# saugns/saugns

Measured on AMD Instinct MI355X. Metric: mono samples/sec/GPU @ N voices (depth-3 FM), higher is better.
Workload: dtype f32 (f64 table interpolation, u32 phase)

## Files before the change

saugns_amd/csrc/engine.cpp:

```cpp
#include <atomic>
#include "engine.h"
#include <algorithm>
#include <exception>
#include <chrono>
#include <stdio.h>
#include <stdlib.h>
#include <string.h>

namespace sauengine {

static const sauProgramIDArr g_no_ids = {0};

static uint64_t ms_to_samples(uint64_t ms, uint64_t srate, int *carry) {
	uint64_t t = ms * srate;
	if (carry) {
		t += *carry;
		*carry = (int)(t % 1000);
	}
	return t / 1000;
}

Engine::~Engine() { delete backend_; }

const char *tune_env(const char *name) {
// ... 210 lines not shown
							err.clear();
						}
					}
				}
				if (vn.shape >= 0) {
					const VoicePlan &sp = shapes_[vn.shape].plan;
					if (plan_check_) {
						VoicePlan chk;
						std::string e2;
						const bool ok = compile_voice_plan(st.ops, vn.carr_op, chk, e2);
						if (!ok || chk.op_ids != shape_ids_ || chk.steps.size() != sp.steps.size() ||
						    memcmp(chk.steps.data(), sp.steps.data(), sp.steps.size() * sizeof(Step)) != 0 ||
						    chk.wave_mask != wmask || chk.n_fast != sp.n_fast || chk.n_fast_full != sp.n_fast_full ||
						    chk.n_slots != sp.n_slots || chk.n_main != sp.n_main || chk.no_fast != sp.no_fast ||
						    chk.static_block != sp.static_block || chk.selfmod != sp.selfmod || chk.n_chain != sp.n_chain ||
						    chk.n_osc != sp.n_osc || chk.has_camods != sp.has_camods || chk.carr_local != sp.carr_local || chk.wide != sp.wide) {
							err = "plan cache: a cached plan differs from a fresh compile (SAU_AMD_PLAN_CHECK)";
							return false;
						}
					}
					vn.plan.steps.clear(); vn.plan.fast_ids.clear(); vn.plan.fast_ids_full.clear();
					vn.plan.op_ids = shape_ids_;
					vn.plan.carr_local = sp.carr_local; vn.plan.n_slots = sp.n_slots; vn.plan.n_main = sp.n_main;
					vn.plan.n_fast = sp.n_fast; vn.plan.n_fast_full = sp.n_fast_full; vn.plan.wave_mask = wmask;
					vn.plan.has_camods = sp.has_camods; vn.plan.no_fast = sp.no_fast; vn.plan.static_block = sp.static_block;
					vn.plan.selfmod = sp.selfmod; vn.plan.n_chain = sp.n_chain; vn.plan.n_osc = sp.n_osc; vn.plan.wide = sp.wide;
					vn.plan.ras_cub = false;
					for (uint32_t id : shape_ids_) if (st.ops[id].ras_cub_seen) vn.plan.ras_cub = true;
					vn.plan.n_steps = (uint32_t)sp.steps.size();
				} else if (!compile_voice_plan(st.ops, vn.carr_op, vn.plan, err)) {
					vn.plan.steps.clear();
					vn.plan.fast_ids.clear();
					vn.plan.fast_ids_full.clear();
					vn.plan.op_ids.clear();
					vn.plan.n_steps = 0;
					if (err != "voice carrier operator was never initialised")
						return false;
					err.clear();
				} else {
					vn.plan.n_steps = (uint32_t)vn.plan.steps.size();
				}
// ... 73 lines not shown
		const sauProgramIDArr *lst = m.mods[use];
		for (uint32_t i = 0; i < count(lst); ++i) {
			const uint32_t o = estimate_sum_levels(st, lst->ids[i], dep, varies, need, nest + 1);
			if (o > out) out = o;
		}
	}
	return out;
}

bool Engine::render_segment(uint32_t len, uint32_t offset, bool stereo, std::string &err) {
	std::vector<VoiceDesc> descs;
	std::vector<SegmentDesc::Stream> sdescs(streams_.size());
	uint32_t n_main = 1, n_fpool = 0, max_ops = 1, n_pan = 0, max_steps = 1, n_fast = 1, n_fast_full = 0;
	uint64_t wave_mask = 0;
	bool maybe_block = false, serial = false, may_scan = false, maybe_cub = false;
	uint32_t sum_levels = 0, n_chain_rows = 0, n_chain_slots = 0, n_inc_rows = 0, n_look_rows = 0, n_may_scan = 0;
	bool chain_rows_padded = false;
	for (size_t s = 0; s < streams_.size(); ++s) {
		Stream &st = streams_[s];
		SegmentDesc::Stream &sd = sdescs[s];
		sd.first_voice = (uint32_t)descs.size();
		sd.amp_scale = st.amp_scale;
		sd.write_len = 0;
		Lattice lat;
		lat.call_len = lat_call_;
		lat.e0 = st.since_event < seg_call_pos_ ? (uint32_t)st.since_event : seg_call_pos_;
		lat.span_left = lat_call_ - seg_call_pos_;
		uint32_t ev_left = 0xffffffffu;
		if (st.event < st.events.size()) {
			const uint32_t wt = st.events[st.event].wait - (st.event_pos - len);
// ... 31 lines not shown
			d.inc_base = 0; d.n_inc = 0;
			d.look_base = 0; d.n_look = 0;
			if (dyn) line_begin(carr.pan, out_len, false, 0.f, lat, 0);
			else line_skip(carr.pan, out_len, lat, 0);
			descs.push_back(d);
			if (out_len > sd.write_len) sd.write_len = out_len;
			n_main = std::max(n_main, vn.plan.n_main);
			if (!vn.plan.no_fast) n_fast = std::max(n_fast, vn.plan.n_fast);
			n_fpool = std::max(n_fpool, vn.plan.n_slots - vn.plan.n_main);
			max_ops = std::max(max_ops, (uint32_t)vn.plan.op_ids.size());
			max_steps = std::max(max_steps, vn.plan.n_steps);
			wave_mask |= vn.plan.wave_mask;
			bool voice_block = vn.plan.static_block;
			if (vn.plan.static_block || vn.plan.no_fast) maybe_block = true;
			if (vn.plan.selfmod) serial = true;
			if (vn.plan.ras_cub && loop_tails_) maybe_cub = true;
			for (uint32_t id : vn.plan.op_ids) {
				OpMirror &m = st.ops[id];
				if (m.goal_seen || (m.line_set & (1u << L_PMA))) { maybe_block = true; voice_block = true; }
				if (m.line_set & (1u << L_PMA)) serial = true;
				if (id != vn.carr_op && !m.time_inf) {
					if (m.time < run_len) maybe_block = true;
					m.time -= std::min(m.time, out_len);
				}
			}
			if (out_len < run_len) maybe_block = true;
			if (voice_block && !vn.plan.no_fast) {
				n_fast_full = std::max(n_fast_full, vn.plan.n_fast_full);
				may_scan = true;
				++n_may_scan;
// ... 64 lines not shown
	seg.streams = sdescs.data(); seg.n_streams = (uint32_t)sdescs.size();
	seg.n_slots = n_main + n_fpool; seg.n_main = n_main; seg.n_fast = n_fast; seg.n_fast_full = n_fast_full; seg.max_ops = max_ops; seg.n_pan_rows = n_pan;
	seg.max_steps = max_steps;
	seg.wave_mask = wave_mask;
	seg.maybe_block = maybe_block;
	seg.serial = serial;
	seg.maybe_cub = maybe_cub;
	seg.may_scan = may_scan;
	seg.sum_levels = sum_levels;
	seg.n_chain_rows = n_chain_rows;
	seg.n_chain_slots = n_chain_slots > n_chain_rows ? n_chain_slots : n_chain_rows;
	seg.n_inc_rows = n_inc_rows;
	seg.n_look_rows = n_look_rows;
	seg.n_may_scan = n_may_scan;
	seg.chain_rows_padded = chain_rows_padded;
	return backend_->render(seg, err);
}

bool Engine::reserve(size_t frames, bool stereo, std::string &err) {
	if (frames > UINT32_MAX) { err = "buffer too long"; return false; }
	if ((uint32_t)frames > reserved_frames_ || (stereo && !reserved_stereo_)) {
		const uint32_t want = std::max((uint32_t)frames, reserved_frames_);
		if (!backend_->reserve_frames(want, stereo || reserved_stereo_, err)) return false;
		reserved_frames_ = want;
		reserved_stereo_ = stereo || reserved_stereo_;
	}
	return true;
}

bool Engine::snapshot(Snapshot &s, int slot, std::string &err) {
// ... 297 lines not shown
```

saugns_amd/csrc/engine.h:

```cpp
#ifndef SAU_ENGINE_H
#define SAU_ENGINE_H

#include "../../include/sau_abi.h"
#include "sau_dev_types.h"
#include "sau_flac.h"
#include "sau_dither.h"
#include <stddef.h>
#include <stdint.h>
#include <stdlib.h>
#include <string>
#include <unordered_map>
#include <vector>

namespace sauengine {

using namespace saudev;

enum SampleFormat : uint8_t { SF_S16 = 0, SF_F32 = 1 };

struct Levels {
	uint64_t frames;
	float peak[2];
	double sum_sq[2];
	uint64_t over[2], full_scale[2], nonfinite[2];
// ... 131 lines not shown
	bool may_scan;
	uint32_t sum_levels = 2;
	uint32_t max_ops;
	uint32_t max_steps;
	uint32_t n_pan_rows;
	uint64_t wave_mask;
	bool maybe_block;
	bool serial;
	bool maybe_cub = false;
	uint32_t n_chain_rows = 0;
	uint32_t n_inc_rows = 0;
	uint32_t n_look_rows = 0;
	uint32_t n_may_scan = 0;
	uint32_t n_chain_slots = 0;
	bool chain_rows_padded = false;
};

inline size_t chain_rows_budget(size_t free_b, unsigned fails) {
	static const long long env_mb = [] {
		const char *v = getenv("SAU_AMD_CHAIN_ROWS_MB");
		return v ? atoll(v) : -1ll;
	}();
	const unsigned sh = fails > 40 ? 40 : fails;
	if (env_mb >= 0) return ((size_t)env_mb << 20) >> sh;
	const size_t dflt = (size_t)24 << 30;
	if (!free_b) return dflt >> sh;
	return (free_b / 8 < dflt ? free_b / 8 : dflt) >> sh;
}

struct BackendConfig {
// ... 163 lines not shown
	std::vector<uint32_t> op_ids;
	uint32_t carr_local = 0;
	uint32_t n_slots = 0;
	uint32_t n_main = 0;
	uint32_t n_fast = 0;
	std::vector<FastIds> fast_ids;
	uint32_t n_fast_full = 0;
	std::vector<FastIds> fast_ids_full;
	uint64_t wave_mask = 0;
	bool has_camods = false;
	bool no_fast = false;
	bool wide = false;
	bool static_block = false;
	bool selfmod = false;
	bool ras_cub = false;
	uint32_t n_chain = 0;
	uint32_t n_osc = 0;
};

bool compile_voice_plan(const std::vector<OpMirror> &ops, uint32_t carrier,
		VoicePlan &out, std::string &err);
bool voice_plan_shape(const std::vector<OpMirror> &ops, uint32_t carrier, std::vector<uint32_t> &tokens,
		std::vector<uint32_t> &op_ids, std::vector<uint32_t> &stamp, uint32_t mark, uint64_t &wave_mask);


constexpr uint32_t CHAIN_SEG = 131072;
const char *tune_env(const char *name);
uint32_t chain_seg_frames(size_t n_chains, size_t budget_bytes);

class Engine {
// ... 161 lines not shown
```

saugns_amd/csrc/hip_backend.hip:

```cpp
#include <hip/hip_runtime.h>
#include "hip_backend.h"
#include "launch_plan.h"
#include "sau_dev_ops.h"
#include "sau_md5.h"
#include <float.h>
#include <stdio.h>
#include <stdlib.h>
#include <string.h>
#include <deque>
#include <map>
#include <memory>
#include <mutex>
#include <string>
#include <type_traits>
#include <vector>

namespace sauhip {

using namespace saudev;
using sauengine::BackendConfig;
using sauengine::tune_env;
using sauengine::SegmentDesc;
using namespace sauplan;

// ... 139 lines not shown
}

static std::mutex &attr_mutex() { static std::mutex *m = new std::mutex; return *m; }
static bool raise_lds_attr(const void *fn, size_t lds, int dev, std::string &err) {
	static std::map<std::pair<const void *, int>, size_t> *slots = new std::map<std::pair<const void *, int>, size_t>;
	std::lock_guard<std::mutex> lk(attr_mutex());
	size_t &configured = (*slots)[std::make_pair(fn, dev & 15)];
	if (lds > configured) {
		hipError_t e = hipFuncSetAttribute(fn, hipFuncAttributeMaxDynamicSharedMemorySize, (int)lds);
		if (e != hipSuccess) { err = std::string("hipFuncSetAttribute: ") + hipGetErrorString(e); return false; }
		configured = lds;
	}
	return true;
}

enum : unsigned { FK_WIDE = 1, FK_TAIL = 2, FK_CUB = 4, FK_INNER = 8, FK_LANEMAJOR = 16, FK_TAB0 = 32 };
static const void *fast_kernel_fn(int build, uint32_t rows, unsigned form) {
	struct Entry { int build; uint32_t rows; unsigned form; const void *fn; };
#define FK(build, form, ...) {build, FK_ROWS(__VA_ARGS__), form, (const void *)fast_kernel<__VA_ARGS__>}
#define FK_ROWS(rows, ...) rows
	static const Entry table[] = {
		FK(0, 0, 2, 0), FK(0, 0, 4, 0), FK(0, 0, 5, 0), FK(0, 0, 6, 0), FK(0, 0, 8, 0),
		FK(1, 0, 2, 1), FK(1, 0, 4, 1),
		FK(2, 0, 2, 2), FK(2, 0, 4, 2), FK(2, 0, 5, 2), FK(2, 0, 6, 2), FK(2, 0, 8, 2),
		FK(3, 0, 4, 3), FK(3, 0, 5, 3), FK(3, 0, 6, 3),
		FK(0, FK_WIDE, 6, 0, false, true), FK(0, FK_WIDE, 8, 0, false, true), FK(0, FK_WIDE, 10, 0, false, true), FK(0, FK_WIDE, 12, 0, false, true),
		FK(2, FK_WIDE | FK_TAIL, 8, 2, false, true, true), FK(2, FK_WIDE, 8, 2, false, true), FK(2, FK_TAIL, 8, 2, false, false, true),
		FK(2, FK_CUB, (int)FAST_CUB_ROWS, 2, true),
		FK(0, FK_WIDE | FK_INNER | FK_LANEMAJOR, 12, 0, false, true, false, true, true), FK(0, FK_WIDE | FK_INNER, 12, 0, false, true, false, true),
#if FK_LM_TAB0
		FK(0, FK_WIDE | FK_INNER | FK_LANEMAJOR | FK_TAB0, 12, 0, false, true, false, true, true, true),
#endif
		FK(0, FK_CUB, (int)FAST_CUB_ROWS, 0, true)};
#undef FK
#undef FK_ROWS
	for (const Entry &e : table)
		if (e.build == build && e.rows == rows && e.form == form) return e.fn;
	return nullptr;
}
#if FK_LM_TAB0
static bool tab0_kernel_ok(const void *fn) {
	static const bool ok = [&] { hipFuncAttributes a; return fn && hipFuncGetAttributes(&a, fn) == hipSuccess && a.sharedSizeBytes == 0; }();
	return ok;
}
#endif
static const void *repair_kernel_fn(uint32_t rows, bool wide) {
// ... 746 lines not shown
			fp.inmix_div_s = k.div.s; fp.inmix_div_m = k.div.m;
			if (k.inmix) {
				fp.inmix_stream = sets_[j.set].mstreams.p;
				fp.inmix_pcm_offset = seg.pcm_offset;
				hipLaunchKernelGGL(premix_kernel, dim3((seg.n_voices + 63) / 64), dim3(64), 0, stream_, fp);
				j.inmix_live = true;
			}
		}
		if (k.inner != INNER_NONE) {
			const bool lm = k.inner == INNER_LANE_MAJOR;
#if FK_LM_TAB0
			const bool tab0 = lm && k.inner_tab0 && tab0_kernel_ok(fast_kernel_fn(0, 12, FK_WIDE | FK_INNER | FK_LANEMAJOR | FK_TAB0));
#else
			const bool tab0 = false;
#endif
			const void *ik = fast_kernel_fn(0, 12, FK_WIDE | FK_INNER | (lm ? FK_LANEMAJOR : 0u) | (tab0 ? FK_TAB0 : 0u));
			if (!ik) { err = "no inner instantiation of fast_kernel for this form"; return false; }
			const size_t lds = k.inner_lds();
			FastParams ep = fp;
			ep.mode = 0; ep.edge_only = 1; ep.dyn_static = 1; ep.dyn_chunks = 2; ep.dyn_small = 0; ep.inmix_flags = 0;
			if (!launch_build(j, err, 0, k.rows, k.grid_edge, &ep, false, true)) j.launched = false;
			fp.mode = 0;
			void *iargs[] = {(void *)&fp};
			if (!raise_lds_attr(ik, lds, dev_, err)) return false;
			if (fp.inmix_flags && !pcm_hazard(err)) return false;
			HIP_OK(hipLaunchKernel(ik, dim3(k.grid), dim3(1024), iargs, lds, stream_));
			if (inner_report_) fprintf(stderr, "[sau-amd] inner: %s, %u voices, %u tables%s\n", lm ? "lane-major" : "row-major", seg.n_voices, k.tabs.n, tab0 ? ", tab0" : "");
		} else {
			if (inner_report_) fprintf(stderr, "[sau-amd] inner: none (rows %u, wide %d, chunks %u), %u voices\n", k.rows, k.wide_cf ? 1 : 0, fp.dyn_chunks, seg.n_voices);
			if (fp.inmix_flags && (!rows_hazard(j, err) || !pcm_hazard(err))) return false;
			launch_fast(j, err, 0);
		}
		fp.dyn_chunks = 0; fp.inmix_flags = 0; fp.dyn_small = 0;
		return true;
	}

	bool launch_cub(Job &j, std::string &err) {
		if (!j.fp.cub_ok) return true;
		const FastPlan &k = j.fk;
		FastParams q = k.main_build == 2 ? j.cfp : j.fp;
		q.n_fast = k.n_fast_cf; q.rows = FAST_CUB_ROWS; q.mode = 0; q.only_multi = 0;
		q.dyn_chunks = k.tasks_cub.dyn_chunks; q.dyn_static = k.tasks_cub.dyn_static;
// ... 1617 lines not shown
```

saugns_amd/csrc/k_fast_group_lm.h:

```cpp
		const int j0 = l * T;
		const int t0 = (int)(cg * GF) - (int)H + j0;
		const uint32_t om = ((1u << T) - 1u) & ~((1u << min(max((int)H - j0, 0), T)) - 1u);
		auto prev32 = [&](const uint32_t *x, int k) -> uint32_t { return k > 0 ? x[k - 1] : lane_prev(x[T - 1]); };
		auto prev64 = [&](const double *x, int k) -> double { return k > 0 ? x[k - 1] : lane_prev(x[T - 1]); };
		const bool quads = ((cg * GF - H) & 3u) == 0;
		auto store_row = [&](float *row, const float *x, const bool nt) {
			uint32_t o = om;
			asm volatile("" : "+v"(o));
			if (quads) {
#pragma unroll
				for (int q = 0; q < T / 4; ++q) {
					const uint32_t oq = (o >> (4 * q)) & 15u;
					if (oq == 15u) {
						const fk_f32x4 v4 = {x[4 * q], x[4 * q + 1], x[4 * q + 2], x[4 * q + 3]};
						fk_f32x4 *p = (fk_f32x4 *)(row + t0 + 4 * q);
						if (nt) FK_VSTORE(p, v4); else *p = v4;
					} else if (oq != 0u) {
#pragma unroll
						for (int u = 0; u < 4; ++u)
							if ((oq >> u) & 1u) { if (nt) FK_VSTORE(&row[t0 + 4 * q + u], x[4 * q + u]); else row[t0 + 4 * q + u] = x[4 * q + u]; }
					}
				}
			} else {
#pragma unroll
				for (int k = 0; k < T; ++k)
					if ((o >> k) & 1u) { if (nt) FK_VSTORE(&row[t0 + k], x[k]); else row[t0 + k] = x[k]; }
			}
		};
		uint32_t held_rows = 0;
		bool held_far = false;
		float blk[T];
		for (uint32_t si = 0; si < n_fsteps; ++si) {
			const FastStep f = load_step_uniform(fsteps + si);
			const uint32_t kind = f.kind & 0xff;
			const uint32_t flags = (f.kind >> 8) & 0xff;
			int t0s = t0;
			asm volatile("" : "+v"(t0s));
			{
				const uint32_t o1 = f.out_off + 1u, p1 = f.pm_off + 1u, q1 = f.fpm_off + 1u, a1 = f.amp_off + 1u;
				uint32_t two = 0;
				if (kind == ST_OSC) two = o1 | a1 | (p1 + q1) | (flags & SF_WAVE_ENV);
				else if (kind == ST_LINE) two = o1;
				else if (kind == ST_VOICE) two = o1 | (p1 << 1);
				else if (kind == ST_LERP) two = 2u;
				if (two > 1u) { zero_acc = 1; continue; }
			}
			if (kind == ST_OSC) {
				const uint32_t type = f.type & 0xff;
				const bool layer = (flags & SF_LAYER) != 0;
				const bool to_voice = ((f.kind >> 16) & OX_VOICE) != 0;
				float s[T];
				if (type == OT_WAVE) {
					const bool has_pm = f.pm_off != ~0u, has_fpm = f.fpm_off != ~0u;
					const int p_min = (int)H - (int)(f.kind >> 24) + 1;
					const int nd = min(max(p_min - j0, 0), T);
					const uint32_t dm = ((1u << T) - 1u) & ~((1u << nd) - 1u);
					bool done = false;
					if (FK_COMMON && f.tab >= 0 && !has_fpm && !(f.ramp & 2)) {
						uint32_t ph[T];
						{
							uint32_t acc = f.phase0 + f.inc * (uint32_t)(t0 + 1);
#pragma unroll
							for (int k = 0; k < T; ++k) { ph[k] = acc; acc += f.inc; }
						}
						bool ok = true;
						if (has_pm) {
							float pm[T];
							bool big = false;
#pragma unroll
							for (int k = 0; k < T; ++k) {
								pm[k] = blk[k];
								big |= !(fabsf(pm[k]) < 0x1p20f);
							}
							ok = !__any(big);
#pragma unroll
							for (int k = 0; k < T; ++k) ph[k] += rint32w_p31_small(pm[k]);
						}
						if (ok) {
							const uint32_t ltab = tabs + (uint32_t)f.tab * FkTab<WIDE>::BYTES;
							static_assert(T % 2 == 0, "pairs of samples");
							auto hermite = [&](auto &&sink) {
// ... 177 lines not shown
								const int j = j0 + (int)__builtin_ctz(held);
								rep[1] = ((uint32_t)(j % 64 - p_min) << 24) | ((uint32_t)(j / 64) << 20) | (si << 12) | (cg & 0xfff);
							}
							const int nf = jm + p_min - j0;
							const bool far = nf <= 0 ? held != 0u : nf < T ? (held >> nf) != 0u : false;
							if (__any(far)) held_far = true;
							if (jm > 0) {
								unsigned long long run = 0;
#pragma unroll
								for (int L = 0; L * T < 64; ++L)
									run |= (unsigned long long)(uint32_t)__builtin_amdgcn_readlane((int)held, L) << (L * T);
								held_rows |= (uint32_t)((run >> p_min) & ((1ull << jm) - 1ull));
							}
						}
					}
				} else if (type == OT_RASEG) {
					const bool rate2x = (f.type >> 17) & 1;
					const float phase_scale = rate2x ? 0x1p31f * 2 : 0x1p31f;
					const RasParams rp = ras_params((uint32_t)f.tab & 0xff, ((uint32_t)f.tab >> 8) & 0xffff,
							f_bits(f.diff_scale), f_bits(f.diff_offset), ((uint32_t)f.tab >> 24) & 0x7f);
					const unsigned long long inc64 = ((unsigned long long)f.prev_phase << 32) | f.inc;
					const unsigned long long cp0 = (unsigned long long)__double_as_longlong(f.prev_Is);
					const bool has_pm = f.pm_off != ~0u, has_fpm = f.fpm_off != ~0u;
#pragma unroll
					for (int k = 0; k < T; ++k) {
						unsigned long long cp = cp0 + inc64 * (unsigned long long)(long long)(t0s + k);
						if (has_pm || has_fpm)
							cp += (unsigned long long)pm_offset(has_pm, has_fpm,
									has_pm ? blk[k] : 0.f,
									has_fpm ? blk[k] : 0.f, f.fc, phase_scale);
						uint32_t cyc;
						float phf;
						ras_split(cp, cyc, phf);
						s[k] = ras_sample(rp, cyc, phf, true, false);
					}
				} else if (type == OT_NOISE) {
					const uint32_t nz = (f.type >> 8) & 0xff;
					const uint32_t n0 = f.phase0;
#pragma unroll
					for (int k = 0; k < T; ++k) {
						const uint32_t n = n0 + (uint32_t)(t0s + k);
						if (nz == NZ_vi) {
							uint32_t s1 = ranfast32(n);
							uint32_t s0 = ranfast32(n - 1);
							s[k] = fscalei((s1 / 2) - (s0 / 2), 0x1p-31f);
						} else if (nz == NZ_bv) {
							int32_t s1 = noise_bv_term(n);
							int32_t s0 = noise_bv_term(n - 1);
							s[k] = (float)(s1 - s0);
						} else {
							s[k] = noise_stateless(nz, n);
						}
					}
				} else {
#pragma unroll
					for (int k = 0; k < T; ++k) s[k] = f.fc;
				}
				float r[T];
				if (f.amp_off != ~0u) {
#pragma unroll
					for (int k = 0; k < T; ++k) r[k] = blk[k];
				} else if (f.ramp & 1) {
					const FastLine fl = load_line_uniform(flines + si);
#pragma unroll
					for (int k = 0; k < T; ++k) r[k] = fast_line_value(fl, t0s + k);
				} else {
#pragma unroll
					for (int k = 0; k < T; ++k) r[k] = f.ac;
				}
				if (layer) {
#pragma unroll
					for (int k = 0; k < T; ++k) r[k] = mix_combine(blk[k], s[k], r[k], false, true);
				} else {
#pragma unroll
					for (int k = 0; k < T; ++k) r[k] = s[k] * r[k];
				}
				if (to_voice) {
					store_row(vrow, r, true);
				} else {
#pragma unroll
					for (int k = 0; k < T; ++k) blk[k] = r[k];
				}
			} else if (kind == ST_LINE) {
				if (f.ramp) {
					FastLine fl;
					fl.goal_len = 0; fl.hold = f.ac; fl.pad = 0;
					fl.sw = sweep_setup(LN_sah, 0.f, 0.f, 0, 1);
					if (f.ramp & 1) fl = load_line_uniform(flines + si);
#pragma unroll
					for (int k = 0; k < T; ++k) blk[k] = fast_line_value(fl, t0s + k);
				} else {
#pragma unroll
					for (int k = 0; k < T; ++k) blk[k] = f.ac;
				}
			} else if (kind == ST_VOICE) {
				store_row(vrow, blk, true);
				if (prow) {
					float x[T];
// ... 25 lines not shown
```

saugns_amd/csrc/k_fast_voice.h:

```cpp
#ifndef FK_TEMPORAL_ROWS
#define FK_VSTORE(p, v) __builtin_nontemporal_store((v), (p))
#else
#define FK_VSTORE(p, v) (*(p) = (v))
#endif
#ifndef FK_TEMPORAL_ROWS
#define FK_CSTORE(p, v) __builtin_nontemporal_store((v), (p))
#define FK_CLOAD(p) __builtin_nontemporal_load(p)
#else
#define FK_CSTORE(p, v) (*(p) = (v))
#define FK_CLOAD(p) (*(p))
#endif

#if FK_LM_ONE_PHASE_SET && !FK_LM_AHEAD
#error "FK_LM_ONE_PHASE_SET needs FK_LM_AHEAD: without its fences the compiler's schedule of the one loop spills (216 VGPRs)"
#endif

__device__ __forceinline__ uint32_t lane_prev(uint32_t x) {
	return (uint32_t)__builtin_amdgcn_update_dpp(0, (int)x, 0x138 , 0xf, 0xf, true);
}
__device__ __forceinline__ double lane_prev(double x) {
	const uint32_t lo = lane_prev((uint32_t)__double2loint(x));
	const uint32_t hi = lane_prev((uint32_t)__double2hiint(x));
	return __hiloint2double((int)hi, (int)lo);
}
// ... 70 lines not shown
			uint2 *d01 = (uint2 *)(lds + (size_t)t * FkTab<WIDE>::BYTES + FkTab<WIDE>::C01);
			for (uint32_t i = tid; i < WAVE_LEN; i += nthreads) d01[i] = ((const uint2 *)s01)[i];
		}
	}
}

__device__ __forceinline__ FastStep load_step_uniform(const FastStep *p) {
	const_u32_ptr q = (const_u32_ptr)(uintptr_t)p;
	union { FastStep s; uint32_t u[20]; } c;
#pragma unroll
	for (int i = 0; i < 20; ++i) c.u[i] = q[i];
	return c.s;
}

template <int T, int SCAN, bool REPAIR = false, bool CUB = false, bool WIDE = false, int SPLIT = 0 , bool TAIL = false,
		bool TAB0 = false >
__device__ __forceinline__ void fast_voice(const FastParams &P, const uint32_t v, const FastInfo &fi,
		float *slots, unsigned long long *carry, const uint32_t tabs , const int l,
		const uint32_t wpv, const uint32_t cstart, unsigned long long *lring = nullptr,
		const uint32_t dyn_c = 0, const uint32_t dyn_k = 0 ,
		const uint32_t vpos = ~0u ,
		const uint32_t wg_waves = 16u ) {
	constexpr int NP = 64 * T;
	(void)NP;
	const uint32_t fast_total = uni(fi.total);
	if (fast_total == 0) return;
	if ((uni(fi.cub) != 0) != CUB) return;
	const VoiceDesc vd = P.voices[v];
	const uint32_t H = uni(fi.H);

	constexpr bool FULL = SCAN == 1;
// ... 272 lines not shown
		if (l == 0) __hip_atomic_fetch_or(&A.ctl[INMIX_CHUNK + INMIX_LINE * (kc - 8) + INMIX_BITS + (j >> 5)], 1u << (j & 31u), __ATOMIC_RELAXED, __HIP_MEMORY_SCOPE_AGENT);
	}
}

#ifndef FK_SPLIT_MASK
#define FK_SPLIT_MASK 9
#endif
#ifndef FK_MINB
#define FK_MINB 1
#endif
#ifdef FK_WAVES_EU
#define FK_ATTR __launch_bounds__(1024) __attribute__((amdgpu_waves_per_eu(FK_WAVES_EU)))
#else
#define FK_ATTR __launch_bounds__(1024, FK_MINB)
#endif
template <int T, int SCAN, bool CUB = false, bool WIDE = false, bool TAIL = false, bool INNER = false, bool LM = false, bool TAB0 = false>
__global__ void FK_ATTR fast_kernel(FastParams P) {
	static_assert(!TAB0 || LM, "the one-table address form exists for the lane-major inner build");
	static_assert(!INNER || (SCAN == 0 && WIDE && T == 12 && !CUB && !TAIL), "the inner-groups-only form exists for the 12-row wide closed-form build");
	static_assert(!LM || INNER, "the lane-major form exists for the inner-groups-only build");
	static_assert(!WIDE || ((SCAN == 0 || SCAN == 2) && !CUB), "only the closed-form and the look-back builds have a wide-table form");
	static_assert(!TAIL || (SCAN == 2 && !CUB && T == 8), "the stream-mixing form exists for the 8-row look-back build");
	constexpr int NP = 64 * T;
	constexpr int W = 16;
	constexpr int SPLIT = INNER ? (LM ? 3 : 2) : (!CUB && ((SCAN == 0 && T == 8 && (FK_SPLIT_MASK & 1)) || (SCAN == 0 && T == 10 && (FK_SPLIT_MASK & 2)) ||
	                                (SCAN == 0 && T == 12 && (FK_SPLIT_MASK & 4)) || (SCAN == 2 && T == 8 && (FK_SPLIT_MASK & 8)))) ? 1 : 0;
	extern __shared__ __align__(16) unsigned char lds[];
	const int tid = threadIdx.x;
	const int w = (int)uni((uint32_t)tid >> 6);
	const int l = tid & 63;
	if (SCAN == 1 && P.mode != 0 && P.mode <= P.sum_levels && P.pass_flags[P.mode - 1] == 0) return;
	if (SCAN == 1 && P.mode == P.sum_levels + 2 && P.pass_flags[FAST_MAX_LEVELS + 1] == 0) return;
	if (SCAN == 1 && P.only_multi && P.pass_flags[FAST_MAX_LEVELS + 2] == 0) return;
// ... 28 lines not shown
		const bool mixing = im && (P.inmix_flags & 32u) && uni(__hip_atomic_load(&P.work_count[1], __ATOMIC_RELAXED, __HIP_MEMORY_SCOPE_AGENT)) == 0;
		for (;;) {
			uint32_t t_ = snext;
			if (counted && !im) { t_ = 0; if (l == 0) t_ = atomicAdd(&P.pass_flags[FAST_DYN_CTR], 1u); }
			if (!CUB && im) {
				const InmixArgs A = inmix_args(NVc);
				const unsigned long long nx = inmix_next(A, mixing ? A.ctl[INMIX_NCH] : K, l);
				t_ = nx == ~0ull ? n_tasks : (uint32_t)nx * K + (uint32_t)(nx >> 32);
			}
			const uint32_t task = uni(t_);
			if (task >= n_tasks) break;
			snext = task + stride;
			const uint32_t vi = task / K;
			const uint32_t v = P.split_cf ? P.vlists[vi] : vi;
			const FastInfo fi = P.info[v];
			fast_voice<T, 0, false, CUB, WIDE, SPLIT, false, TAB0>(P, v, fi, slots, carry, tabs, l, 1u, 0u, nullptr, task - vi * K, K);
			if (!CUB && mixing) {
				const InmixArgs A = inmix_args(NVc);
				inmix_after(A, task - vi * K, vi, l);
			}
		}
		return;
	}
	const uint32_t g = blockIdx.x * W + (uint32_t)w;
	const uint32_t total_waves = gridDim.x * W;
	if (SCAN == 2) {
		const uint32_t NVl = P.pass_flags[FAST_LK_COUNT];
		uint32_t wpv = P.look_wpv;
		if (P.look_words_real) {
			wpv = total_waves / NVl;
			if (wpv > P.look_groups) wpv = P.look_groups;
// ... 135 lines not shown
```

saugns_amd/csrc/launch_plan.h:

```cpp
#ifndef SAU_LAUNCH_PLAN_H
#define SAU_LAUNCH_PLAN_H

#include "engine.h"
#include "mix_overlap.h"
#include "sau_dev_math.h"
#include <string.h>

namespace sauplan {

using namespace saudev;
using sauengine::SegmentDesc;

#ifndef FK_GRID
#define FK_GRID 256
#endif
constexpr uint32_t FAST_TAB_BYTES = (uint32_t)(WAVE_LEN * (sizeof(HerpC23) + sizeof(HerpC01))), FAST_TAB_BYTES_WIDE = 65536u;
constexpr uint32_t FAST_MAX_SCAN = 8;
constexpr uint32_t LOOK_LDS_BYTES = FAST_MAX_SCAN * 2 * 64 * sizeof(unsigned long long);
constexpr uint32_t FAST_MAX_LEVELS = 3;
constexpr uint32_t FAST_CUB_ROWS = 4;
constexpr uint32_t FAST_LISTS = 5;
constexpr uint32_t INMIX_NSMALL = 8;
#ifndef SAU_CHAIN_BATCH_FRAMES
#define SAU_CHAIN_BATCH_FRAMES 32
// ... 37 lines not shown
	uint32_t lean_rows = 6;
	bool dyn = true;
	uint32_t dyn_groups = 12;
	uint32_t dyn_floor = 24;
	uint32_t dyn_min_tasks = 2;
	bool xcd_queues = true;
	bool inmix = true;
	uint32_t inmix_min_voices = 64;
	uint32_t inmix_min_steps = 2;
	bool inmix_taper = false;
	uint32_t inmix_at = 13;
	uint32_t inmix_at_lm = 15;
	bool inmix_dry = false;
	bool inner = true;
	bool lanemajor = true;
	bool duo = true;
	uint32_t duo_lw = 0, duo_prio = 0;
	bool tailmix = false;
	bool mix_few = true;
	bool early_mix = true;
	bool mix64 = true;
	bool poison = false;
	bool mix_overlap = true;
	bool mix_overlap_shared = false;
	uint32_t mix_overlap_mb = 4096;
	bool mix_overlap_fail = false;
};

inline Tuning tuning_from_env(const char *(*env)(const char *)) {
	Tuning t;
// ... 38 lines not shown
	t.lean = off("SAU_AMD_NO_LEAN");
	num("SAU_AMD_LEAN_ROWS", t.lean_rows);
	t.dyn = off("SAU_AMD_NO_DYN");
	at_least_1("SAU_AMD_DYN_GROUPS", t.dyn_groups);
	at_least_1("SAU_AMD_DYN_FLOOR", t.dyn_floor);
	at_least_1("SAU_AMD_DYN_MIN_TASKS", t.dyn_min_tasks);
	t.xcd_queues = off("SAU_AMD_NO_XCD_QUEUES");
	t.inmix = off("SAU_AMD_NO_INMIX");
	num("SAU_AMD_INMIX_MIN_VOICES", t.inmix_min_voices);
	num("SAU_AMD_INMIX_MIN_STEPS", t.inmix_min_steps);
	t.inmix_taper = !off("SAU_AMD_INMIX_TAPER");
	if (const char *ia = env("SAU_AMD_INMIX_AT")) t.inmix_at = t.inmix_at_lm = (uint32_t)atoi(ia) & 15u;
	t.inmix_dry = !off("SAU_AMD_INMIX_DRY");
	t.inner = off("SAU_AMD_NO_INNER");
	t.lanemajor = off("SAU_AMD_NO_LANEMAJOR");
	t.duo = off("SAU_AMD_NO_DUO");
	if (const char *lw = env("SAU_AMD_DUO_LW")) t.duo_lw = (uint32_t)atoi(lw) & 15u;
	if (const char *pr = env("SAU_AMD_DUO_PRIO")) t.duo_prio = (uint32_t)atoi(pr) & 7u;
	t.tailmix = !off("SAU_AMD_TAILMIX");
	t.mix_few = off("SAU_AMD_NO_MIX_FEW");
	t.early_mix = off("SAU_AMD_NO_EARLY_MIX");
	t.mix64 = off("SAU_AMD_NO_MIX64");
	t.poison = !off("SAU_AMD_POISON");
	t.mix_overlap = off("SAU_AMD_NO_MIX_OVERLAP");
	t.mix_overlap_shared = !off("SAU_AMD_MIX_OVERLAP_SHARED");
	if (const char *mb = env("SAU_AMD_MIX_OVERLAP_MB")) { const long n = atol(mb); t.mix_overlap_mb = n < 0 ? 0u : n > 0x7fffffffl ? 0x7fffffffu : (uint32_t)n; }
	t.mix_overlap_fail = !off("SAU_AMD_MIX_OVERLAP_FAIL");
	return t;
}

// ... 168 lines not shown
	if (d.s == 0) return q;
	const uint32_t t = (uint32_t)(((unsigned long long)q * d.m) >> 32);
	return (t + ((q - t) >> 1)) >> (d.s - 1);
}

#ifndef FK_LM_ONE_PHASE_SET
#define FK_LM_ONE_PHASE_SET 1
#endif
#ifndef FK_LM_TAB0
#define FK_LM_TAB0 0
#endif
#ifndef FK_LM_AHEAD
#define FK_LM_AHEAD 1
#endif
constexpr bool FK_LM_SHORT_TASKS = FK_LM_ONE_PHASE_SET && FK_LM_AHEAD;
enum Inner : uint32_t { INNER_NONE = 0, INNER_ROW_MAJOR = 1, INNER_LANE_MAJOR = 2 };
enum Mixer : uint32_t { MIX_NONE = 0, MIX_FEW_F32, MIX_F32, MIX_FEW, MIX_64, MIX_256 };

struct FastPlan {
	bool use_fast = false;
	bool seq_ok = false;
	bool look_split = false;
	int main_build = 0;
	uint32_t fmax_steps = 0, n_fast = 0, n_fast_cf = 0;
	uint32_t rows = 2;
	uint32_t rows_multi = 2;
	uint32_t rows_cf = 2;
	uint32_t rows_lean = 4;
	bool lean_on = false;
	TableMap tabs;
// ... 13 lines not shown
	bool inc_rows = false;
	uint32_t inc_stride = 0;
	bool chains = false;
	uint32_t chain_stride = 0, chain_grid = 0;
	TableMap ctabs;
	ChainChunks chunks;
	uint32_t pass_grid = 0;
	bool early_mix = false;
	bool split_cf = false, duo = false, tailmix = false;
	bool queues = false;
	bool inmix = false;
	uint32_t inmix_flags = 0;
	MagicDiv div;
	Inner inner = INNER_NONE;
	bool inner_tab0 = false;
	Tasks tasks, tasks_cf, tasks_cub;
	uint32_t groups = 0, groups_cf = 0;
	uint32_t grid = 1, grid_cf = 1, grid_look = 1, grid_edge = 1, grid_cub = 1, grid_repair = 1;
	uint32_t rows_repair = 2;

	void drop_chains() { chains = false; lean_on = false; }
	size_t launch_lds(int build, uint32_t r, bool wide, bool cf = false) const {
		return tabs.n * (size_t)(wide ? FAST_TAB_BYTES_WIDE : FAST_TAB_BYTES) + 16 * buf_area(cf ? n_fast_cf : n_fast, r, fmax_steps) +
			(build == 2 ? LOOK_LDS_BYTES : 0);
	}
	size_t inner_lds() const {
		return inner == INNER_LANE_MAJOR ? tabs.n * (size_t)FAST_TAB_BYTES_WIDE : launch_lds(0, rows, true);
	}
};

// ... 112 lines not shown
			const uint32_t small = G / 4 ? G / 4 : 1;
			if (p.groups >= 32 * G + INMIX_NSMALL * small) {
				p.tasks.dyn_small = small;
				p.tasks.dyn_chunks = (p.groups - INMIX_NSMALL * small + G - 1) / G + INMIX_NSMALL;
			}
		}
		p.div = magic_div(seg.n_voices);
		p.inmix = tun.inmix && !in.f32 && seg.n_streams == 1 && in.max_write && seg.n_voices >= tun.inmix_min_voices &&
			seg.max_steps >= tun.inmix_min_steps && in.row_stride < (1u << 24);
		if (p.inmix)
			p.inmix_flags = 64u | 32u | (seg.stereo ? 1u : 0u) | (seg.swap_bytes ? 2u : 0u) | (tun.inmix_dry ? 4u : 0u) | ((tun.inmix_at & 15u) << 8);
	}
	if (tun.inner && p.main_build == 0 && p.wide_cf && p.rows == 12 && p.tasks.dyn_chunks >= 3)
		p.inner = tun.lanemajor && p.n_fast == 1 ? INNER_LANE_MAJOR : INNER_ROW_MAJOR;
	p.inner_tab0 = p.inner == INNER_LANE_MAJOR && p.tabs.n == 1;
	if (FK_LM_SHORT_TASKS && p.inmix && p.inner == INNER_LANE_MAJOR) p.inmix_flags = (p.inmix_flags & ~(15u << 8)) | ((tun.inmix_at_lm & 15u) << 8);
	p.grid_edge = wave_grid(2ull * seg.n_voices, dev.fk_grid);
}

inline FastPlan plan_fast(const SegmentDesc &seg, const Tuning &tun, const DeviceLimits &dev, const PlanInputs &in) {
	FastPlan p;
	plan_rows(p, seg, tun, dev);
	plan_sums(p, seg, tun, dev);
	p.groups = row_groups(seg.len, p.rows);
	p.grid = group_grid(seg.n_voices, p.groups, dev.fk_grid);
	plan_chains(p, seg, tun, dev, in);
	if (p.use_fast && p.main_build == 2) plan_split(p, seg, tun, dev, in);
	if (p.use_fast && !p.scan) plan_closed_form(p, seg, tun, dev, in);
	const uint32_t g4 = row_groups(seg.len, FAST_CUB_ROWS);
	p.grid_cub = group_grid(seg.n_voices, g4, dev.fk_grid);
// ... 322 lines not shown
```

saugns_amd/csrc/plan.cpp:

```cpp
#include "engine.h"
#include <unordered_map>

namespace sauengine {

namespace {

constexpr uint32_t WIDE_MAIN_MAX = 4096, WIDE_FREQ_MAX = 4095;

struct Compiler {
	const std::vector<OpMirror> &ops;
	VoicePlan &out;
	std::string &err;
	std::vector<uint32_t> path;
	std::unordered_map<uint32_t, uint32_t> local;
	std::vector<WideStep> wsteps;
	std::vector<bool> used = std::vector<bool>(0x10000, false);
	uint32_t high = 0;
	uint32_t high_f = 0;
	bool failed = false;

	Compiler(const std::vector<OpMirror> &o, VoicePlan &p, std::string &e)
		: ops(o), out(p), err(e) { used[SCRATCH_SLOT] = true; }

	uint16_t alloc() {
// ... 299 lines not shown
		}
		if (st.kind == ST_SMLINE) { out.static_block = true; out.selfmod = true; }
		if (st.kind == ST_LINE && st.which == L_FREQ && (st.flags & SF_FORCE)) out.static_block = true;
	}
	{
		std::vector<uint8_t> seen(out.op_ids.size(), 0);
		for (const Step &st : out.steps) {
			if (st.kind == ST_WIDE) continue;
			if (st.kind == ST_ZERO) out.no_fast = true;
			if (st.kind == ST_OSC) {
				if (seen[st.op]) out.no_fast = true;
				seen[st.op] = 1;
			}
		}
	}
	out.fast_ids.assign(out.steps.size(), FastIds());
	out.fast_ids_full.assign(out.steps.size(), FastIds());
	out.n_fast = out.n_fast_full = 0xffffffffu;
	if (!out.wide) {
		out.n_fast = fast_slot_compact(out.steps.data(), (uint32_t)out.steps.size(),
				out.steps.empty() ? nullptr : out.fast_ids.data(), false);
		uint8_t ramped[256];
		for (size_t i = 0; i < 256; ++i) {
			ramped[i] = 7;
			if (i < out.op_ids.size()) {
				const OpMirror &m = ops[out.op_ids[i]];
				ramped[i] = (uint8_t)((m.freq_goal_seen ? 1 : 0) | (m.goal_seen ? 2 : 0) | (m.freq_ratio_seen ? 4 : 0));
			}
		}
		static const bool lean = !tune_env("SAU_AMD_NO_LEAN_IDS");
// ... 13 lines not shown
```

Before: 254.4 million.

## Add wave-only specialization of lane-major inner fast kernel

The plan compiler now marks voice plans made only of plain wave oscillators (no amp/fpm mods, layering, envelopes, or ramps). When every voice in a segment qualifies, the host selects a new lane-major kernel instantiation compiled with those branches removed. That kernel also computes phase-modulated phases directly from a base plus per-row increment. This cuts branches, register pressure and dead paths in the hot loop, at the cost of another template instantiation and extra plan-classification logic that must stay correct.

```diff
diff --git a/saugns_amd/csrc/engine.cpp b/saugns_amd/csrc/engine.cpp
--- a/saugns_amd/csrc/engine.cpp
+++ b/saugns_amd/csrc/engine.cpp
@@ -248,7 +248,8 @@
 						    chk.wave_mask != wmask || chk.n_fast != sp.n_fast || chk.n_fast_full != sp.n_fast_full ||
 						    chk.n_slots != sp.n_slots || chk.n_main != sp.n_main || chk.no_fast != sp.no_fast ||
 						    chk.static_block != sp.static_block || chk.selfmod != sp.selfmod || chk.n_chain != sp.n_chain ||
-						    chk.n_osc != sp.n_osc || chk.has_camods != sp.has_camods || chk.carr_local != sp.carr_local || chk.wide != sp.wide) {
+						    chk.n_osc != sp.n_osc || chk.has_camods != sp.has_camods || chk.carr_local != sp.carr_local || chk.wide != sp.wide ||
+						    chk.wave_only != sp.wave_only) {
 							err = "plan cache: a cached plan differs from a fresh compile (SAU_AMD_PLAN_CHECK)";
 							return false;
 						}
@@ -259,6 +260,7 @@
 					vn.plan.n_fast = sp.n_fast; vn.plan.n_fast_full = sp.n_fast_full; vn.plan.wave_mask = wmask;
 					vn.plan.has_camods = sp.has_camods; vn.plan.no_fast = sp.no_fast; vn.plan.static_block = sp.static_block;
 					vn.plan.selfmod = sp.selfmod; vn.plan.n_chain = sp.n_chain; vn.plan.n_osc = sp.n_osc; vn.plan.wide = sp.wide;
+					vn.plan.wave_only = sp.wave_only;
 					vn.plan.ras_cub = false;
 					for (uint32_t id : shape_ids_) if (st.ops[id].ras_cub_seen) vn.plan.ras_cub = true;
 					vn.plan.n_steps = (uint32_t)sp.steps.size();
@@ -362,6 +364,7 @@
 	uint32_t n_main = 1, n_fpool = 0, max_ops = 1, n_pan = 0, max_steps = 1, n_fast = 1, n_fast_full = 0;
 	uint64_t wave_mask = 0;
 	bool maybe_block = false, serial = false, may_scan = false, maybe_cub = false;
+	bool wave_only = true;
 	uint32_t sum_levels = 0, n_chain_rows = 0, n_chain_slots = 0, n_inc_rows = 0, n_look_rows = 0, n_may_scan = 0;
 	bool chain_rows_padded = false;
 	for (size_t s = 0; s < streams_.size(); ++s) {
@@ -423,6 +426,7 @@
 			bool voice_block = vn.plan.static_block;
 			if (vn.plan.static_block || vn.plan.no_fast) maybe_block = true;
 			if (vn.plan.selfmod) serial = true;
+			if (!vn.plan.wave_only) wave_only = false;
 			if (vn.plan.ras_cub && loop_tails_) maybe_cub = true;
 			for (uint32_t id : vn.plan.op_ids) {
 				OpMirror &m = st.ops[id];
@@ -517,6 +521,7 @@
 	seg.n_look_rows = n_look_rows;
 	seg.n_may_scan = n_may_scan;
 	seg.chain_rows_padded = chain_rows_padded;
+	seg.wave_only = wave_only && !maybe_block && !may_scan;
 	return backend_->render(seg, err);
 }
 
diff --git a/saugns_amd/csrc/engine.h b/saugns_amd/csrc/engine.h
--- a/saugns_amd/csrc/engine.h
+++ b/saugns_amd/csrc/engine.h
@@ -169,6 +169,7 @@
 	uint32_t n_may_scan = 0;
 	uint32_t n_chain_slots = 0;
 	bool chain_rows_padded = false;
+	bool wave_only = false;
 };
 
 inline size_t chain_rows_budget(size_t free_b, unsigned fails) {
@@ -362,6 +363,7 @@
 	bool static_block = false;
 	bool selfmod = false;
 	bool ras_cub = false;
+	bool wave_only = false;
 	uint32_t n_chain = 0;
 	uint32_t n_osc = 0;
 };
diff --git a/saugns_amd/csrc/hip_backend.hip b/saugns_amd/csrc/hip_backend.hip
--- a/saugns_amd/csrc/hip_backend.hip
+++ b/saugns_amd/csrc/hip_backend.hip
@@ -177,7 +177,7 @@
 	return true;
 }
 
-enum : unsigned { FK_WIDE = 1, FK_TAIL = 2, FK_CUB = 4, FK_INNER = 8, FK_LANEMAJOR = 16, FK_TAB0 = 32 };
+enum : unsigned { FK_WIDE = 1, FK_TAIL = 2, FK_CUB = 4, FK_INNER = 8, FK_LANEMAJOR = 16, FK_TAB0 = 32, FK_WONLY = 64 };
 static const void *fast_kernel_fn(int build, uint32_t rows, unsigned form) {
 	struct Entry { int build; uint32_t rows; unsigned form; const void *fn; };
 #define FK(build, form, ...) {build, FK_ROWS(__VA_ARGS__), form, (const void *)fast_kernel<__VA_ARGS__>}
@@ -193,6 +193,9 @@
 		FK(0, FK_WIDE | FK_INNER | FK_LANEMAJOR, 12, 0, false, true, false, true, true), FK(0, FK_WIDE | FK_INNER, 12, 0, false, true, false, true),
 #if FK_LM_TAB0
 		FK(0, FK_WIDE | FK_INNER | FK_LANEMAJOR | FK_TAB0, 12, 0, false, true, false, true, true, true),
+#endif
+#if FK_LM_WONLY
+		FK(0, FK_WIDE | FK_INNER | FK_LANEMAJOR | FK_WONLY, 12, 0, false, true, false, true, true, false, true),
 #endif
 		FK(0, FK_CUB, (int)FAST_CUB_ROWS, 0, true)};
 #undef FK
@@ -969,7 +972,8 @@
 #else
 			const bool tab0 = false;
 #endif
-			const void *ik = fast_kernel_fn(0, 12, FK_WIDE | FK_INNER | (lm ? FK_LANEMAJOR : 0u) | (tab0 ? FK_TAB0 : 0u));
+			const bool wonly = FK_LM_WONLY && lm && k.inner_wonly && !tab0;
+			const void *ik = fast_kernel_fn(0, 12, FK_WIDE | FK_INNER | (lm ? FK_LANEMAJOR : 0u) | (tab0 ? FK_TAB0 : 0u) | (wonly ? FK_WONLY : 0u));
 			if (!ik) { err = "no inner instantiation of fast_kernel for this form"; return false; }
 			const size_t lds = k.inner_lds();
 			FastParams ep = fp;
@@ -980,7 +984,7 @@
 			if (!raise_lds_attr(ik, lds, dev_, err)) return false;
 			if (fp.inmix_flags && !pcm_hazard(err)) return false;
 			HIP_OK(hipLaunchKernel(ik, dim3(k.grid), dim3(1024), iargs, lds, stream_));
-			if (inner_report_) fprintf(stderr, "[sau-amd] inner: %s, %u voices, %u tables%s\n", lm ? "lane-major" : "row-major", seg.n_voices, k.tabs.n, tab0 ? ", tab0" : "");
+			if (inner_report_) fprintf(stderr, "[sau-amd] inner: %s, %u voices, %u tables%s\n", lm ? "lane-major" : "row-major", seg.n_voices, k.tabs.n, tab0 ? ", tab0" : wonly ? ", wonly" : "");
 		} else {
 			if (inner_report_) fprintf(stderr, "[sau-amd] inner: none (rows %u, wide %d, chunks %u), %u voices\n", k.rows, k.wide_cf ? 1 : 0, fp.dyn_chunks, seg.n_voices);
 			if (fp.inmix_flags && (!rows_hazard(j, err) || !pcm_hazard(err))) return false;
diff --git a/saugns_amd/csrc/k_fast_group_lm.h b/saugns_amd/csrc/k_fast_group_lm.h
--- a/saugns_amd/csrc/k_fast_group_lm.h
+++ b/saugns_amd/csrc/k_fast_group_lm.h
@@ -35,10 +35,17 @@
 			const uint32_t kind = f.kind & 0xff;
 			const uint32_t flags = (f.kind >> 8) & 0xff;
 			int t0s = t0;
-			asm volatile("" : "+v"(t0s));
+			if (!WONLY) asm volatile("" : "+v"(t0s));
 			{
 				const uint32_t o1 = f.out_off + 1u, p1 = f.pm_off + 1u, q1 = f.fpm_off + 1u, a1 = f.amp_off + 1u;
 				uint32_t two = 0;
+				if (WONLY) {
+					static_assert(OT_AMP == 0 && OT_WAVE == 2, "the types as bits");
+					const uint32_t ty = f.type & 0xff & ~(uint32_t)OT_WAVE;
+					if (kind == ST_OSC) two = o1 | p1 | ((a1 | q1 | (flags & (SF_WAVE_ENV | SF_LAYER)) | (f.ramp & 1u) | ty) << 1);
+					else if (kind == ST_VOICE) two = o1 | (p1 << 1);
+					else two = 2u;
+				} else
 				if (kind == ST_OSC) two = o1 | a1 | (p1 + q1) | (flags & SF_WAVE_ENV);
 				else if (kind == ST_LINE) two = o1;
 				else if (kind == ST_VOICE) two = o1 | (p1 << 1);
@@ -51,20 +58,34 @@
 				const bool to_voice = ((f.kind >> 16) & OX_VOICE) != 0;
 				float s[T];
 				if (type == OT_WAVE) {
-					const bool has_pm = f.pm_off != ~0u, has_fpm = f.fpm_off != ~0u;
+					const bool has_pm = f.pm_off != ~0u, has_fpm = !WONLY && f.fpm_off != ~0u;
 					const int p_min = (int)H - (int)(f.kind >> 24) + 1;
 					const int nd = min(max(p_min - j0, 0), T);
 					const uint32_t dm = ((1u << T) - 1u) & ~((1u << nd) - 1u);
 					bool done = false;
 					if (FK_COMMON && f.tab >= 0 && !has_fpm && !(f.ramp & 2)) {
 						uint32_t ph[T];
-						{
+						bool ok = true;
+						if (WONLY && FK_LM_WONLY_ADD3) {
+							const uint32_t base = f.phase0 + f.inc * (uint32_t)(t0 + 1);
+							if (has_pm) {
+								bool big = false;
+#pragma unroll
+								for (int k = 0; k < T; ++k) big |= !(fabsf(blk[k]) < 0x1p20f);
+								ok = !__any(big);
+#pragma unroll
+								for (int k = 0; k < T; ++k) ph[k] = base + (uint32_t)k * f.inc + rint32w_p31_small(blk[k]);
+							} else {
+								uint32_t acc = base;
+#pragma unroll
+								for (int k = 0; k < T; ++k) { ph[k] = acc; acc += f.inc; }
+							}
+						} else {
 							uint32_t acc = f.phase0 + f.inc * (uint32_t)(t0 + 1);
 #pragma unroll
 							for (int k = 0; k < T; ++k) { ph[k] = acc; acc += f.inc; }
 						}
-						bool ok = true;
-						if (has_pm) {
+						if (!(WONLY && FK_LM_WONLY_ADD3) && has_pm) {
 							float pm[T];
 							bool big = false;
 #pragma unroll
@@ -272,7 +293,7 @@
 							}
 						}
 					}
-				} else if (type == OT_RASEG) {
+				} else if (!WONLY && type == OT_RASEG) {
 					const bool rate2x = (f.type >> 17) & 1;
 					const float phase_scale = rate2x ? 0x1p31f * 2 : 0x1p31f;
 					const RasParams rp = ras_params((uint32_t)f.tab & 0xff, ((uint32_t)f.tab >> 8) & 0xffff,
@@ -292,7 +313,7 @@
 						ras_split(cp, cyc, phf);
 						s[k] = ras_sample(rp, cyc, phf, true, false);
 					}
-				} else if (type == OT_NOISE) {
+				} else if (!WONLY && type == OT_NOISE) {
 					const uint32_t nz = (f.type >> 8) & 0xff;
 					const uint32_t n0 = f.phase0;
 #pragma unroll
@@ -314,11 +335,23 @@
 #pragma unroll
 					for (int k = 0; k < T; ++k) s[k] = f.fc;
 				}
+				if (WONLY && FK_LM_WONLY_INPLACE) {
+					if (to_voice) {
+						float x[T];
+#pragma unroll
+						for (int k = 0; k < T; ++k) x[k] = s[k] * f.ac;
+						store_row(vrow, x, true);
+					} else {
+#pragma unroll
+						for (int k = 0; k < T; ++k) blk[k] = s[k] * f.ac;
+					}
+					continue;
+				}
 				float r[T];
-				if (f.amp_off != ~0u) {
+				if (!WONLY && f.amp_off != ~0u) {
 #pragma unroll
 					for (int k = 0; k < T; ++k) r[k] = blk[k];
-				} else if (f.ramp & 1) {
+				} else if (!WONLY && (f.ramp & 1)) {
 					const FastLine fl = load_line_uniform(flines + si);
 #pragma unroll
 					for (int k = 0; k < T; ++k) r[k] = fast_line_value(fl, t0s + k);
@@ -326,7 +359,7 @@
 #pragma unroll
 					for (int k = 0; k < T; ++k) r[k] = f.ac;
 				}
-				if (layer) {
+				if (!WONLY && layer) {
 #pragma unroll
 					for (int k = 0; k < T; ++k) r[k] = mix_combine(blk[k], s[k], r[k], false, true);
 				} else {
@@ -339,7 +372,7 @@
 #pragma unroll
 					for (int k = 0; k < T; ++k) blk[k] = r[k];
 				}
-			} else if (kind == ST_LINE) {
+			} else if (!WONLY && kind == ST_LINE) {
 				if (f.ramp) {
 					FastLine fl;
 					fl.goal_len = 0; fl.hold = f.ac; fl.pad = 0;
diff --git a/saugns_amd/csrc/k_fast_voice.h b/saugns_amd/csrc/k_fast_voice.h
--- a/saugns_amd/csrc/k_fast_voice.h
+++ b/saugns_amd/csrc/k_fast_voice.h
@@ -108,7 +108,8 @@
 }
 
 template <int T, int SCAN, bool REPAIR = false, bool CUB = false, bool WIDE = false, int SPLIT = 0 , bool TAIL = false,
-		bool TAB0 = false >
+		bool TAB0 = false ,
+		bool WONLY = false >
 __device__ __forceinline__ void fast_voice(const FastParams &P, const uint32_t v, const FastInfo &fi,
 		float *slots, unsigned long long *carry, const uint32_t tabs , const int l,
 		const uint32_t wpv, const uint32_t cstart, unsigned long long *lring = nullptr,
@@ -411,9 +412,11 @@
 #else
 #define FK_ATTR __launch_bounds__(1024, FK_MINB)
 #endif
-template <int T, int SCAN, bool CUB = false, bool WIDE = false, bool TAIL = false, bool INNER = false, bool LM = false, bool TAB0 = false>
+template <int T, int SCAN, bool CUB = false, bool WIDE = false, bool TAIL = false, bool INNER = false, bool LM = false, bool TAB0 = false,
+		bool WONLY = false>
 __global__ void FK_ATTR fast_kernel(FastParams P) {
 	static_assert(!TAB0 || LM, "the one-table address form exists for the lane-major inner build");
+	static_assert(!WONLY || LM, "the wave-only form exists for the lane-major inner build");
 	static_assert(!INNER || (SCAN == 0 && WIDE && T == 12 && !CUB && !TAIL), "the inner-groups-only form exists for the 12-row wide closed-form build");
 	static_assert(!LM || INNER, "the lane-major form exists for the inner-groups-only build");
 	static_assert(!WIDE || ((SCAN == 0 || SCAN == 2) && !CUB), "only the closed-form and the look-back builds have a wide-table form");
@@ -472,7 +475,7 @@
 			const uint32_t vi = task / K;
 			const uint32_t v = P.split_cf ? P.vlists[vi] : vi;
 			const FastInfo fi = P.info[v];
-			fast_voice<T, 0, false, CUB, WIDE, SPLIT, false, TAB0>(P, v, fi, slots, carry, tabs, l, 1u, 0u, nullptr, task - vi * K, K);
+			fast_voice<T, 0, false, CUB, WIDE, SPLIT, false, TAB0, WONLY>(P, v, fi, slots, carry, tabs, l, 1u, 0u, nullptr, task - vi * K, K);
 			if (!CUB && mixing) {
 				const InmixArgs A = inmix_args(NVc);
 				inmix_after(A, task - vi * K, vi, l);
diff --git a/saugns_amd/csrc/launch_plan.h b/saugns_amd/csrc/launch_plan.h
--- a/saugns_amd/csrc/launch_plan.h
+++ b/saugns_amd/csrc/launch_plan.h
@@ -75,6 +75,8 @@
 	bool inmix_dry = false;
 	bool inner = true;
 	bool lanemajor = true;
+	bool inner_wonly = true;
+	bool inner_wonly_force = false;
 	bool duo = true;
 	uint32_t duo_lw = 0, duo_prio = 0;
 	bool tailmix = false;
@@ -143,6 +145,8 @@
 	t.inmix_dry = !off("SAU_AMD_INMIX_DRY");
 	t.inner = off("SAU_AMD_NO_INNER");
 	t.lanemajor = off("SAU_AMD_NO_LANEMAJOR");
+	t.inner_wonly = off("SAU_AMD_NO_INNER_WONLY");
+	t.inner_wonly_force = !off("SAU_AMD_INNER_WONLY_FORCE");
 	t.duo = off("SAU_AMD_NO_DUO");
 	if (const char *lw = env("SAU_AMD_DUO_LW")) t.duo_lw = (uint32_t)atoi(lw) & 15u;
 	if (const char *pr = env("SAU_AMD_DUO_PRIO")) t.duo_prio = (uint32_t)atoi(pr) & 7u;
@@ -341,6 +345,15 @@
 #define FK_LM_AHEAD 1
 #endif
 constexpr bool FK_LM_SHORT_TASKS = FK_LM_ONE_PHASE_SET && FK_LM_AHEAD;
+#ifndef FK_LM_WONLY
+#define FK_LM_WONLY 1
+#endif
+#ifndef FK_LM_WONLY_ADD3
+#define FK_LM_WONLY_ADD3 1
+#endif
+#ifndef FK_LM_WONLY_INPLACE
+#define FK_LM_WONLY_INPLACE 0
+#endif
 enum Inner : uint32_t { INNER_NONE = 0, INNER_ROW_MAJOR = 1, INNER_LANE_MAJOR = 2 };
 enum Mixer : uint32_t { MIX_NONE = 0, MIX_FEW_F32, MIX_F32, MIX_FEW, MIX_64, MIX_256 };
 
@@ -384,6 +397,7 @@
 	MagicDiv div;
 	Inner inner = INNER_NONE;
 	bool inner_tab0 = false;
+	bool inner_wonly = false;
 	Tasks tasks, tasks_cf, tasks_cub;
 	uint32_t groups = 0, groups_cf = 0;
 	uint32_t grid = 1, grid_cf = 1, grid_look = 1, grid_edge = 1, grid_cub = 1, grid_repair = 1;
@@ -526,6 +540,7 @@
 	if (tun.inner && p.main_build == 0 && p.wide_cf && p.rows == 12 && p.tasks.dyn_chunks >= 3)
 		p.inner = tun.lanemajor && p.n_fast == 1 ? INNER_LANE_MAJOR : INNER_ROW_MAJOR;
 	p.inner_tab0 = p.inner == INNER_LANE_MAJOR && p.tabs.n == 1;
+	p.inner_wonly = FK_LM_WONLY && p.inner == INNER_LANE_MAJOR && ((tun.inner_wonly && seg.wave_only) || tun.inner_wonly_force);
 	if (FK_LM_SHORT_TASKS && p.inmix && p.inner == INNER_LANE_MAJOR) p.inmix_flags = (p.inmix_flags & ~(15u << 8)) | ((tun.inmix_at_lm & 15u) << 8);
 	p.grid_edge = wave_grid(2ull * seg.n_voices, dev.fk_grid);
 }
diff --git a/saugns_amd/csrc/plan.cpp b/saugns_amd/csrc/plan.cpp
--- a/saugns_amd/csrc/plan.cpp
+++ b/saugns_amd/csrc/plan.cpp
@@ -337,6 +337,15 @@
 			}
 		}
 	}
+	out.wave_only = !out.wide && !out.no_fast && !out.static_block && !out.has_camods && !out.steps.empty();
+	for (const Step &st : out.steps) {
+		if (!out.wave_only) break;
+		if (st.kind == ST_LINE && st.which == L_FREQ && !(st.flags & SF_FORCE) && st.out >= FSLOT_BASE) continue;
+		if (st.kind != ST_OSC || (st.flags & (SF_LAYER | SF_WAVE_ENV)) || (st.freq != NO_SLOT && st.freq < FSLOT_BASE) || st.fpm != NO_SLOT ||
+		    st.amp != NO_SLOT || st.sm != NO_SLOT || st.op >= out.op_ids.size()) { out.wave_only = false; break; }
+		const OpMirror &om = ops[out.op_ids[st.op]];
+		if (om.type != SAU_POPT_N_wave || om.goal_seen || (om.line_set & (1u << L_PMA))) out.wave_only = false;
+	}
 	out.fast_ids.assign(out.steps.size(), FastIds());
 	out.fast_ids_full.assign(out.steps.size(), FastIds());
 	out.n_fast = out.n_fast_full = 0xffffffffu;
```

Result: faster. 264.7 million (median of 6 runs) (+4.1%).
